# m4drat/wtf

Measured on AMD Instinct MI355X. Metric: execs/sec + emulated instr/s per node (tlv_server, HEVD) at 1/2/4/8 GPUs, higher is better.
Workload: dtype u64

## Files before the change

include/wtfgpu.h:

```cpp
#ifndef WTFGPU_H
#define WTFGPU_H

#include <stdint.h>
#include <stddef.h>

#ifdef __cplusplus
extern "C" {
#endif

#define WTFGPU_ABI_VERSION 4
#define WTFGPU_PAGE_SIZE 4096u

#define WTFGPU_OK 0
#define WTFGPU_ERR_INVALID (-1)
#define WTFGPU_ERR_NODEV (-2)
#define WTFGPU_ERR_OOM (-3)
#define WTFGPU_ERR_HIP (-4)
#define WTFGPU_ERR_STATE (-5)
#define WTFGPU_ERR_TRANSLATE (-6)

enum wtfgpu_status {
  WTFGPU_RUNNING = 0,
  WTFGPU_EXIT_BREAKPOINT = 1,
  WTFGPU_EXIT_TIMEOUT = 2,
// ... 57 lines not shown
  uint64_t zmmh[16][4];
  uint64_t zmm_hi[16][8];
  uint64_t k[8];
} wtfgpu_regs_t;

typedef struct wtfgpu_exit {
  uint32_t status;
  uint32_t vector;
  uint32_t error;
  uint32_t opcode;
  uint64_t addr;
  uint64_t rip;
  uint64_t icount;
} wtfgpu_exit_t;

typedef struct wtfgpu_run_stats {
  uint64_t kernel_launches;
  uint64_t group_steps;
  uint64_t lane_retired;
  double kernel_ms;
} wtfgpu_run_stats_t;

typedef struct wtfgpu_ctx wtfgpu_ctx;

int wtfgpu_abi_version(void);
int wtfgpu_device_count(void);
int wtfgpu_create(int device, wtfgpu_ctx **out);
int wtfgpu_destroy(wtfgpu_ctx *ctx);
void *wtfgpu_stream(wtfgpu_ctx *ctx);
int wtfgpu_select_queue(wtfgpu_ctx *ctx, uint32_t queue);
// ... 68 lines not shown
                      const wtfgpu_regs_t *in);
int wtfgpu_read_gprs(wtfgpu_ctx *ctx, uint32_t first, uint32_t count, uint64_t *out18);
int wtfgpu_write_gprs(wtfgpu_ctx *ctx, uint32_t first, uint32_t count, const uint64_t *in18);

int wtfgpu_read_exits(wtfgpu_ctx *ctx, uint32_t first, uint32_t count, wtfgpu_exit_t *out);
int wtfgpu_resume(wtfgpu_ctx *ctx, const uint32_t *lanes, uint32_t n, const uint8_t *skip_bp);
int wtfgpu_stop(wtfgpu_ctx *ctx, const uint32_t *lanes, uint32_t n, uint32_t status);

int wtfgpu_run(wtfgpu_ctx *ctx, uint32_t first, uint32_t count, uint64_t max_steps,
               wtfgpu_run_stats_t *stats);
int wtfgpu_run_async(wtfgpu_ctx *ctx, uint32_t first, uint32_t count, uint64_t max_steps);
int wtfgpu_run_wait(wtfgpu_ctx *ctx, wtfgpu_run_stats_t *stats);

int wtfgpu_prefetch_results(wtfgpu_ctx *ctx, uint32_t first, uint32_t count, wtfgpu_exit_t *exits,
                            uint64_t *bytes, uint32_t *dirty, uint64_t *stop_args);
int wtfgpu_prefetch_coverage(wtfgpu_ctx *ctx, uint32_t first, uint32_t count, uint64_t *hdr);
int wtfgpu_prefetched_coverage(wtfgpu_ctx *ctx, uint32_t *out_lanes, uint64_t *out_rips, uint64_t n);
int wtfgpu_clear_coverage_lanes(wtfgpu_ctx *ctx, const uint32_t *lanes, uint32_t n);

int wtfgpu_lane_translate(wtfgpu_ctx *ctx, uint32_t lane, uint64_t gva, uint64_t *gpa);
int wtfgpu_lane_read_phys(wtfgpu_ctx *ctx, uint32_t lane, uint64_t gpa, void *buf, uint64_t len);
int wtfgpu_lane_write_phys(wtfgpu_ctx *ctx, uint32_t lane, uint64_t gpa, const void *buf,
                           uint64_t len);
int wtfgpu_lane_read_virt(wtfgpu_ctx *ctx, uint32_t lane, uint64_t gva, void *buf, uint64_t len);
int wtfgpu_lane_write_virt(wtfgpu_ctx *ctx, uint32_t lane, uint64_t gva, const void *buf,
                           uint64_t len);

typedef struct wtfgpu_write {
  uint32_t lane;
  uint32_t len;
  uint64_t gva;
// ... 56 lines not shown
```

wtf_amd/abi.py:

```python
from __future__ import annotations

import ctypes as C
import os

HERE = os.path.dirname(os.path.abspath(__file__))
LIB_PATH = os.environ.get("WTFGPU_LIB") or os.path.join(HERE, "csrc", "libwtfgpu.so")
HOST_LIB_PATH = os.path.join(HERE, "host", "libwtf_host.so")

RUNNING, EXIT_BREAKPOINT, EXIT_TIMEOUT, EXIT_INT3, EXIT_HLT, EXIT_FAULT, EXIT_UNIMPLEMENTED, \
    EXIT_CR3, EXIT_OVERLAY_FULL, EXIT_STOPPED, EXIT_IDLE, EXIT_STOP_OK, EXIT_FEED_FAULT, EXIT_STOP_ARGS = range(14)
STATUS_NAMES = ["running", "breakpoint", "timeout", "int3", "hlt", "fault", "unimplemented",
                "cr3", "overlay_full", "stopped", "idle", "stop_ok", "feed_fault"]


class Seg(C.Structure):
    _fields_ = [("base", C.c_uint64), ("limit", C.c_uint32), ("selector", C.c_uint16),
                ("attr", C.c_uint16), ("present", C.c_uint8), ("pad", C.c_uint8 * 7)]


class Regs(C.Structure):
    _fields_ = [
        ("gpr", C.c_uint64 * 16), ("rip", C.c_uint64), ("rflags", C.c_uint64),
        ("cr0", C.c_uint64), ("cr2", C.c_uint64), ("cr3", C.c_uint64), ("cr4", C.c_uint64),
        ("cr8", C.c_uint64), ("efer", C.c_uint64), ("xcr0", C.c_uint64),
# ... 5 lines not shown
        ("idtr_limit", C.c_uint32), ("mxcsr", C.c_uint32), ("mxcsr_mask", C.c_uint32),
        ("fpcw", C.c_uint16), ("fpsw", C.c_uint16), ("fptw", C.c_uint16), ("fpop", C.c_uint16),
        ("pad0", C.c_uint32), ("fpst", C.c_uint64 * 8), ("xmm", (C.c_uint64 * 2) * 16),
        ("ymmh", (C.c_uint64 * 2) * 16), ("fpse", C.c_uint16 * 8),
        ("zmmh", (C.c_uint64 * 4) * 16), ("zmm_hi", (C.c_uint64 * 8) * 16), ("k", C.c_uint64 * 8),
    ]


class Exit(C.Structure):
    _fields_ = [("status", C.c_uint32), ("vector", C.c_uint32), ("error", C.c_uint32),
                ("opcode", C.c_uint32), ("addr", C.c_uint64), ("rip", C.c_uint64),
                ("icount", C.c_uint64)]

    def tuple(self):
        return (self.status, self.vector, self.error, self.addr, self.rip, self.icount)


class RunStats(C.Structure):
    _fields_ = [("kernel_launches", C.c_uint64), ("group_steps", C.c_uint64),
                ("lane_retired", C.c_uint64), ("kernel_ms", C.c_double)]


class BpAction(C.Structure):
    _fields_ = [("gva", C.c_uint64), ("kind", C.c_uint32), ("pad", C.c_uint32),
                ("value", C.c_uint64), ("gprs", C.c_uint64 * 17)]


BPACT_HOST, BPACT_RETURN, BPACT_SET_GPRS, BPACT_FEED = 0, 1, 2, 3
ATTRIB_ALL = 1

# ... 57 lines not shown
        "wtfgpu_apply_phys_writes": ([P, C.POINTER(Write), U32, C.c_char_p, U64, C.POINTER(I32)], C.c_int),
        "wtfgpu_restore_lanes": ([P, C.POINTER(U32), U32], C.c_int),
        "wtfgpu_set_initial_state": ([P, C.POINTER(Regs)], C.c_int),
        "wtfgpu_set_limit": ([P, U64], C.c_int),
        "wtfgpu_set_regroup": ([P, U64], C.c_int),
        "wtfgpu_set_edges": ([P, C.c_int], C.c_int),
        "wtfgpu_set_trace": ([P, U32], C.c_int),
        "wtfgpu_read_trace": ([P, U32, C.POINTER(U64), U64, C.POINTER(U64)], C.c_int),
        "wtfgpu_read_stop_args": ([P, C.POINTER(U32), U32, C.POINTER(U64)], C.c_int),
        "wtfgpu_select_queue": ([P, U32], C.c_int),
        "wtfgpu_lane_seeds": ([P, C.POINTER(U32), U32, C.POINTER(U64), C.c_int], C.c_int),
        "wtfgpu_run_async": ([P, U32, U32, U64], C.c_int),
        "wtfgpu_run_wait": ([P, C.POINTER(RunStats)], C.c_int),
        "wtfgpu_prefetch_results": ([P, U32, U32, C.POINTER(Exit), C.POINTER(U64), C.POINTER(U32), C.POINTER(U64)],
                                    C.c_int),
        "wtfgpu_prefetch_coverage": ([P, U32, U32, C.POINTER(U64)], C.c_int),
        "wtfgpu_prefetched_coverage": ([P, C.POINTER(U32), C.POINTER(U64), U64], C.c_int),
        "wtfgpu_clear_coverage_lanes": ([P, C.POINTER(U32), U32], C.c_int),
        "wtfgpu_set_breakpoints": ([P, C.POINTER(U64), U32], C.c_int),
        "wtfgpu_set_breakpoint_actions": ([P, C.POINTER(BpAction), U32], C.c_int),
        "wtfgpu_set_feed": ([P, U32, U32, C.POINTER(U64), C.c_char_p, C.c_char_p, U64], C.c_int),
        "wtfgpu_set_code_pages": ([P, C.POINTER(U64), U32], C.c_int),
        "wtfgpu_restore": ([P, U32, U32], C.c_int),
        "wtfgpu_read_regs": ([P, U32, U32, C.POINTER(Regs)], C.c_int),
        "wtfgpu_write_regs": ([P, U32, U32, C.POINTER(Regs)], C.c_int),
        "wtfgpu_read_gprs": ([P, U32, U32, C.POINTER(U64)], C.c_int),
        "wtfgpu_write_gprs": ([P, U32, U32, C.POINTER(U64)], C.c_int),
        "wtfgpu_read_exits": ([P, U32, U32, C.POINTER(Exit)], C.c_int),
        "wtfgpu_resume": ([P, C.POINTER(U32), U32, C.POINTER(C.c_uint8)], C.c_int),
        "wtfgpu_inject_fault": ([P, C.POINTER(U32), U32, U32, U32, C.POINTER(U64), C.POINTER(C.c_int32)], C.c_int),
# ... 37 lines not shown
```

wtf_amd/csrc/engine.hip:

```cpp
#include <hip/hip_runtime.h>
#include <hipcub/device/device_radix_sort.hpp>
#include <hipcub/device/device_scan.hpp>

#include <algorithm>
#include <cstddef>
#include <cstdio>
#include <cstdlib>
#include <cstring>
#include <new>
#include <vector>

#include "engine_run.h"
#include "engine_kernels.h"
#include "engine_ptmark.h"

using namespace wtfgpu_dev;

#define HIPCHK(x)                                                                        \
  do {                                                                                   \
    hipError_t e_ = (x);                                                                 \
    if (e_ != hipSuccess) {                                                              \
      fprintf(stderr, "wtfgpu: %s failed: %s (%s:%d)\n", #x, hipGetErrorString(e_), __FILE__, \
              __LINE__);                                                                 \
      return WTFGPU_ERR_HIP;                                                             \
// ... 9 lines not shown
  u64 stage_bytes = 0;
  u64 *d_stat = nullptr;
  hipEvent_t ev0 = nullptr, ev1 = nullptr;
  u32 *d_rkeys = nullptr, *d_rkeys2 = nullptr, *d_rlanes = nullptr;
  void *d_rtemp = nullptr;
  size_t rtemp_bytes = 0;
  u32 async_launches = 0;
  u8 rg_used = 2;
  u8 *h_ring = nullptr;
  u64 ring_cap = 0, ring_off = 0;
  wtfgpu_exit_t *d_exq = nullptr;
  u64 exq_cap = 0;
  u8 *d_pcov = nullptr;
  hipEvent_t ev_pre = nullptr;
  bool pre_valid = false;
};

struct wtfgpu_ctx {
  int device = 0;
  Dev P{};
  u8 *d_pool = nullptr;
  u32 *d_pfnmap = nullptr;
  u32 *d_ptbits = nullptr;
  u64 npool = 0;
  u64 *d_gpr = nullptr, *d_rip = nullptr, *d_rflags = nullptr, *d_fsb = nullptr, *d_gsb = nullptr,
      *d_icount = nullptr, *d_nbytes = nullptr;
  u32 *d_status = nullptr, *d_lflags = nullptr, *d_ovcount = nullptr, *d_ovgpfn = nullptr;
  ExitInfo *d_exinfo = nullptr;
  LaneSys *d_sys = nullptr;
  u32 *d_guc = nullptr;
// ... 77 lines not shown
int ensure_scratch(wtfgpu_ctx *c, u64 bytes) {
  QueueRes &q = *c->q;
  if (q.scratch_bytes >= bytes) return WTFGPU_OK;
  const u64 want = std::max<u64>(std::max<u64>(bytes, 2 * q.scratch_bytes), 1ull << 20);
  if (q.d_scratch) HIPCHK(hipFreeAsync(q.d_scratch, q.stream));
  q.d_scratch = nullptr;
  q.scratch_bytes = 0;
  if (hipMallocAsync((void **)&q.d_scratch, want, q.stream) != hipSuccess) return WTFGPU_ERR_OOM;
  q.scratch_bytes = want;
  return WTFGPU_OK;
}

u8 *ring_put(wtfgpu_ctx *c, const void *src, u64 bytes) {
  QueueRes &q = *c->q;
  const u64 need = (bytes + 255) & ~255ull;
  if (q.ring_off + need > q.ring_cap) {
    if (hipStreamSynchronize(q.stream) != hipSuccess) return nullptr;
    q.ring_off = 0;
    if (need > q.ring_cap) {
      if (q.h_ring) (void)hipHostFree(q.h_ring);
      q.h_ring = nullptr;
      q.ring_cap = 0;
      const u64 want = std::max<u64>(need * 2, 4ull << 20);
      if (hipHostMalloc((void **)&q.h_ring, want, hipHostMallocDefault) != hipSuccess) return nullptr;
      q.ring_cap = want;
    }
  }
  u8 *p = q.h_ring + q.ring_off;
  if (src && bytes) memcpy(p, src, bytes);
  q.ring_off += need;
  return p;
}
void ring_reset(wtfgpu_ctx *c) { c->q->ring_off = 0; }

int queue_create(QueueRes &q, u32 index) {
  q.index = index;
  HIPCHK(hipStreamCreateWithFlags(&q.stream, hipStreamNonBlocking));
  HIPCHK(hipEventCreate(&q.ev0));
  HIPCHK(hipEventCreate(&q.ev1));
  HIPCHK(hipEventCreateWithFlags(&q.ev_pre, hipEventDisableTiming));
  if (dalloc(&q.d_stat, STAT_N)) return WTFGPU_ERR_OOM;
  return WTFGPU_OK;
}
void regroup_free(QueueRes &q) {
  dfree(q.d_rkeys);
  dfree(q.d_rkeys2);
  dfree(q.d_rlanes);
  dfree(q.d_rtemp);
  q.rtemp_bytes = 0;
}
void queue_destroy(QueueRes &q) {
  if (q.stream) (void)hipStreamSynchronize(q.stream);
  regroup_free(q);
  dfree(q.d_stat);
  dfree(q.d_scratch);
  dfree(q.d_exq);
  dfree(q.d_pcov);
  if (q.h_stage) (void)hipHostFree(q.h_stage);
  q.h_stage = nullptr;
  if (q.h_ring) (void)hipHostFree(q.h_ring);
  q.h_ring = nullptr;
  if (q.ev_pre) (void)hipEventDestroy(q.ev_pre);
  if (q.ev0) (void)hipEventDestroy(q.ev0);
  if (q.ev1) (void)hipEventDestroy(q.ev1);
  if (q.stream) (void)hipStreamDestroy(q.stream);
  q = QueueRes{};
}

u64 hmix(u64 x) {
  x ^= x >> 33;
  x *= 0xff51afd7ed558ccdull;
  x ^= x >> 33;
  x *= 0xc4ceb9fe1a85ec53ull;
  x ^= x >> 33;
  return x;
}

// ... 1057 lines not shown
  if (!lanes_ok(c, first, count) || (first % c->P.lpw) || max_steps == 0 || max_steps > (1ull << 32))
    return WTFGPU_ERR_INVALID;
  if (!c->P.pool) return WTFGPU_ERR_STATE;
  if (c->q->async_launches) return WTFGPU_ERR_STATE;
  HIPCHK(hipSetDevice(c->device));
  const u64 regroup = regroup_now(c, count);
  const u64 chunk = regroup ? regroup : max_steps;
  if (regroup)
    if (int rc = regroup_buffers(c)) return rc;
  const Dev Q = run_params(c, regroup != 0);
  HIPCHK(hipEventRecord(c->q->ev_pre, c->q->stream));
  c->q->pre_valid = true;
  u64 done = 0;
  u32 k = 0;
  if (int rc = queue_launches(c, Q, first, count, chunk, max_steps, ~0ull, regroup != 0, done, k)) return rc;
  c->q->async_launches = k;
  return WTFGPU_OK;
}

int wtfgpu_run_wait(wtfgpu_ctx *c, wtfgpu_run_stats_t *stats) {
  if (!c) return WTFGPU_ERR_INVALID;
  wtfgpu_run_stats_t st{};
  if (c->q->async_launches) {
    HIPCHK(hipSetDevice(c->device));
    u64 running = 0;
    if (int rc = collect_stats(c, c->q->async_launches, st, running)) return rc;
    ring_reset(c);
    c->q->async_launches = 0;
    regroup_observe(c, st.group_steps, st.lane_retired);
  }
  if (stats) *stats = st;
  return WTFGPU_OK;
}

int wtfgpu_prefetch_results(wtfgpu_ctx *c, uint32_t first, uint32_t count, wtfgpu_exit_t *exits, uint64_t *bytes,
                            uint32_t *dirty, uint64_t *stop_args) {
  if (!lanes_ok(c, first, count) || !exits) return WTFGPU_ERR_INVALID;
  if (count == 0) return WTFGPU_OK;
  HIPCHK(hipSetDevice(c->device));
  if (c->q->exq_cap < count) {
    if (c->q->d_exq) HIPCHK(hipFreeAsync(c->q->d_exq, c->q->stream));
    c->q->d_exq = nullptr;
    c->q->exq_cap = 0;
    if (hipMallocAsync((void **)&c->q->d_exq, (u64)count * sizeof(wtfgpu_exit_t), c->q->stream) != hipSuccess)
      return WTFGPU_ERR_OOM;
    c->q->exq_cap = count;
  }
  k_pack_exits<<<(count + 255) / 256, 256, 0, c->q->stream>>>(c->P, first, count, c->q->d_exq);
  HIPCHK(hipGetLastError());
  HIPCHK(hipMemcpyAsync(exits, c->q->d_exq, (u64)count * sizeof(wtfgpu_exit_t), hipMemcpyDeviceToHost, c->q->stream));
  if (bytes) HIPCHK(hipMemcpyAsync(bytes, c->d_nbytes + first, (u64)count * 8, hipMemcpyDeviceToHost, c->q->stream));
  if (dirty) HIPCHK(hipMemcpyAsync(dirty, c->d_ovcount + first, (u64)count * 4, hipMemcpyDeviceToHost, c->q->stream));
  if (stop_args && c->d_stopargs)
    HIPCHK(hipMemcpyAsync(stop_args, c->d_stopargs + (u64)first * 6, (u64)count * 48, hipMemcpyDeviceToHost,
                          c->q->stream));
  return WTFGPU_OK;
}

constexpr u64 kPcovCap = 1ull << 22;
constexpr u64 kPcovLanes = 256, kPcovRips = kPcovLanes + kPcovCap * 4;

int wtfgpu_prefetch_coverage(wtfgpu_ctx *c, uint32_t first, uint32_t count, uint64_t *hdr) {
  if (!lanes_ok(c, first, count) || !hdr) return WTFGPU_ERR_INVALID;
  if (!c->d_covrip || count == 0) {
    hdr[0] = hdr[1] = 0;
    return WTFGPU_ERR_STATE;
  }
  HIPCHK(hipSetDevice(c->device));
  if (!c->q->d_pcov && hipMallocAsync((void **)&c->q->d_pcov, kPcovRips + kPcovCap * 8, c->q->stream) != hipSuccess) {
    c->q->d_pcov = nullptr;
    return WTFGPU_ERR_OOM;
  }
  HIPCHK(hipMemsetAsync(c->q->d_pcov, 0, 16, c->q->stream));
  k_cov_collect_stopped<<<(count + 3) / 4, 256, 0, c->q->stream>>>(
      c->P, first, count, (u32 *)(c->q->d_pcov + kPcovLanes), (u64 *)(c->q->d_pcov + kPcovRips), kPcovCap,
      (unsigned long long *)c->q->d_pcov, (u32 *)(c->q->d_pcov + 8));
  HIPCHK(hipGetLastError());
  HIPCHK(hipMemcpyAsync(hdr, c->q->d_pcov, 16, hipMemcpyDeviceToHost, c->q->stream));
  return WTFGPU_OK;
}

int wtfgpu_prefetched_coverage(wtfgpu_ctx *c, uint32_t *out_lanes, uint64_t *out_rips, uint64_t n) {
  if (!c || (n && (!out_lanes || !out_rips)) || n > kPcovCap || (n && !c->q->d_pcov)) return WTFGPU_ERR_INVALID;
  if (n == 0) return WTFGPU_OK;
  HIPCHK(hipSetDevice(c->device));
  HIPCHK(hipMemcpyAsync(out_lanes, c->q->d_pcov + kPcovLanes, n * 4, hipMemcpyDeviceToHost, c->q->stream));
  HIPCHK(hipMemcpyAsync(out_rips, c->q->d_pcov + kPcovRips, n * 8, hipMemcpyDeviceToHost, c->q->stream));
  HIPCHK(hipStreamSynchronize(c->q->stream));
  return WTFGPU_OK;
}

int wtfgpu_clear_coverage_lanes(wtfgpu_ctx *c, const uint32_t *lanes, uint32_t n) {
  if (!c || (n && !lanes)) return WTFGPU_ERR_INVALID;
// ... 646 lines not shown
```

wtf_amd/csrc/engine_device.h:

```cpp
#pragma once
#ifndef WTFGPU_HOST_SIM
#include <hip/hip_runtime.h>
#else
#include "../../tests/native/host_sim_shim.h"
#endif
#include <stdint.h>
#include "../../include/wtfgpu.h"

namespace wtfgpu_dev {

typedef uint64_t u64;
typedef uint32_t u32;
typedef uint16_t u16;
typedef uint8_t u8;
typedef int64_t i64;
typedef int32_t i32;

constexpr u64 F_CF = 0x1, F_PF = 0x4, F_AF = 0x10, F_ZF = 0x40, F_SF = 0x80, F_TF = 0x100,
              F_IF = 0x200, F_DF = 0x400, F_OF = 0x800;
constexpr u64 F_STATUS = F_CF | F_PF | F_AF | F_ZF | F_SF | F_OF;
constexpr u64 EMPTY_KEY = ~0ull;

constexpr u64 T_W = 1, T_U = 2, T_NX = 4, T_PRIV = 8, T_PT = 16;
constexpr int TLB_N = 4;
// ... 2 lines not shown
  u64 cr0, cr3, cr4, efer;
  u64 star, lstar, sfmask, kgs;
  u64 idtr, tss, cr2;
  u64 deliv_icount;
  u32 idtr_limit, pad;
  u32 cpl;
  u16 cs, ss;
};

struct LaneTlb {
  u64 tv[TLB_N], td[TLB_N];
  u64 cvpn, cptr, bloom;
  u32 tnext, pad;
};

struct ExitInfo {
  u32 vector, error, opcode, cpl;
  u64 addr;
};

struct Dev {
  const u8 *pool;
  const u32 *pfn_map;
  u64 pfn_map_len;
  u64 npool;
  const u32 *ptbits;
  u32 nlanes;
  u32 K;
  u32 lpw;
  u64 *gpr;
  u64 *rip, *rflags, *fs_base, *gs_base, *icount, *nbytes;
  u32 *status, *lflags;
  ExitInfo *exinfo;
  LaneSys *sys;
// ... 85 lines not shown
```

wtf_amd/host/gpu_backend.cc:

```cpp
#include "gpu_backend.h"
#include "module_instances.h"

#include <algorithm>
#include <chrono>
#include <cstdio>
#include <cstring>

#include "host_pool.h"

#include "blake3_lite.h"

namespace wtfgpu_host {

thread_local uint32_t GpuBackend_t::cur_ = 0;
thread_local uint64_t GpuBackend_t::servicing_bp_ = ~0ull;
thread_local uint64_t GpuBackend_t::servicing_sp_ = ~0ull;
thread_local bool GpuBackend_t::scouting_ = false;

namespace {
constexpr uint64_t kFeedRegion = 16384;
using Clock = std::chrono::steady_clock;
double ms_since(Clock::time_point t0) {
  return std::chrono::duration<double, std::milli>(Clock::now() - t0).count();
}
// ... 15 lines not shown
    case Registers_t::R12: return WTFGPU_R12;
    case Registers_t::R13: return WTFGPU_R13;
    case Registers_t::R14: return WTFGPU_R14;
    case Registers_t::R15: return WTFGPU_R15;
    case Registers_t::Rip: return 16;
    case Registers_t::Rflags: return 17;
    default: return -1;
  }
}

}

GpuBackend_t::GpuBackend_t() = default;
GpuBackend_t::~GpuBackend_t() {
  for (Part &P : parts_)
    for (void *p : {(void *)P.pin, (void *)P.ex, (void *)P.nb, (void *)P.dc, (void *)P.sargs, (void *)P.cov_hdr})
      if (p) wtfgpu_host_free(ctx_, p);
  if (wpin_) wtfgpu_host_free(ctx_, wpin_);
  if (ctx_) wtfgpu_destroy(ctx_);
}

bool GpuBackend_t::LoadDump(const std::string &dump_path) { return dump_.Parse(dump_path); }

bool GpuBackend_t::Initialize(const Options_t &Opts, const CpuState_t &CpuState) {
  if (dump_.PageCount() == 0 && !Opts.DumpPath.empty() && !LoadDump(Opts.DumpPath.string())) {
    printf("Failed to parse the dump %s\n", Opts.DumpPath.string().c_str());
    return false;
  }
  if (wtfgpu_create(Opts.GpuDevice, &ctx_) != WTFGPU_OK) {
    printf("wtfgpu_create(%d) failed\n", Opts.GpuDevice);
    return false;
// ... 1357 lines not shown

uint32_t GpuBackend_t::FreeLanes() const {
  if (busy_.empty()) return parts_n() > 1 ? nlanes_ / 2 : nlanes_;
  const Part &P = parts_[next_part_];
  if (P.launched) return P.hi - P.lo;
  return (uint32_t)P.free.size();
}

uint32_t GpuBackend_t::parts_n() const {
  if (!parts_.empty()) return (uint32_t)parts_.size();
  const char *e = getenv("WTFGPU_STREAM_PARTS");
  const uint32_t want = e ? (uint32_t)atoi(e) : 2;
  return (want >= 2 && nlanes_ >= 256 && nlanes_ % 128 == 0) ? 2 : 1;
}

bool GpuBackend_t::StreamStep(const Target_t &Target, const std::vector<StreamTestcase_t> &In, uint64_t Slice,
                              std::vector<StreamResult_t> &Out, ModuleSlots *Slots, size_t *Taken) {
  const auto t0 = Clock::now();
  if (Taken) *Taken = 0;
  if (busy_.empty()) {
    busy_.assign(nlanes_, 0);
    tag_.assign(nlanes_, 0);
    tc_bytes_.assign(nlanes_, 0);
    lres_.assign(nlanes_, LaneResult{});
    plain_.assign(nlanes_, 0);
    const uint32_t n = parts_n();
    done_.assign((nlanes_ + n - 1) / n + 1, 0);
    parts_.assign(n, Part{});
    for (uint32_t p = 0; p < n; p++) {
      Part &Q = parts_[p];
      Q.lo = (uint32_t)((uint64_t)nlanes_ * p / n);
      Q.hi = (uint32_t)((uint64_t)nlanes_ * (p + 1) / n);
      Q.free.resize(Q.hi - Q.lo);
      for (uint32_t l = Q.lo; l < Q.hi; l++) Q.free[l - Q.lo] = l;
    }
    std::vector<uint32_t> all(nlanes_);
    for (uint32_t l = 0; l < nlanes_; l++) all[l] = l;
    if (wtfgpu_stop(ctx_, all.data(), nlanes_, WTFGPU_EXIT_IDLE)) return false;
  }
  const bool pipelined = parts_.size() > 1;
  const uint32_t pi = next_part_;
  next_part_ = (next_part_ + 1) % (uint32_t)parts_.size();
  Part &P = parts_[pi];
  if (pipelined && wtfgpu_select_queue(ctx_, pi)) return false;
  if (pipelined && P.launched && !harvest_part(P, Target, Out, Slots)) return false;
  const auto ti = Clock::now();
  stats_.harvest_ms += std::chrono::duration<double, std::milli>(ti - t0).count();
  std::vector<uint32_t> &fresh = fresh_;
  {
    const size_t take = std::min(In.size(), P.free.size());
    fresh.assign(P.free.begin(), P.free.begin() + (std::ptrdiff_t)take);
    P.free.erase(P.free.begin(), P.free.begin() + (std::ptrdiff_t)take);
  }
  if (Taken) *Taken = fresh.size();
  stats_.fresh_ms += ms_since(ti);
  if (!fresh.empty()) {
    if (wtfgpu_restore_lanes(ctx_, fresh.data(), (uint32_t)fresh.size())) return false;
    stats_.restore_dev_ms += ms_since(ti);
    const size_t n = fresh.size();
// ... 8 lines not shown
    }
    HostPool::Get().For(chunks, 1, [&](size_t c) {
      RefillChunk &C = rchunks_[c];
      C.call.clear();
      C.pre.clear();
      C.bytes = 0;
      const size_t hi = std::min(n, (c + 1) * kChunk);
      for (size_t i = c * kChunk; i < hi; i++) {
        const uint32_t l = fresh[i];
        if (touched_[l]) reset_view(l);
        PrepFeed f{};
        busy_[l] = 1;
        tag_[l] = In[i].tag;
        tc_bytes_[l] = In[i].size;
        const StreamTestcase_t &T = In[i];
        bool prepared = true;
        switch (T.prep) {
          case PreparedInsert_t::Call: prepared = false; break;
          case PreparedInsert_t::Failed:
            view(l).result = Crash_t("insert-testcase-failed");
            C.pre.push_back(l);
            break;
          case PreparedInsert_t::Nothing: break;
          case PreparedInsert_t::Feed:
            if (!feed_action_ || T.prep_size > kFeedRegion)
              prepared = false;
            else
              f = PrepFeed{T.prep_data, (uint32_t)T.prep_size, 1, 0};
            break;
          case PreparedInsert_t::Insert:
            if (!insert_action_ || T.size + 4 > kFeedRegion)
              prepared = false;
            else
              f = PrepFeed{T.data, (uint32_t)T.size, 1, 1};
            break;
        }
        pf_[l] = f;
        flen_[i] = f.has ? f.len + (f.ins ? 4 : 0) : 0;
        fhas_[i] = f.has;
        C.bytes += flen_[i];
        if (!prepared) {
          C.call.push_back((uint32_t)i);
          continue;
        }
        if (Slots) Slots->ResetLane(l);
      }
    }, n >= 512);
    recycle_arenas();
    const auto tm = Clock::now();
    stats_.restore_ms += std::chrono::duration<double, std::milli>(tm - ti).count();
// ... 24 lines not shown
      for (size_t k = 0; k < call_.size(); k++) {
        const uint32_t i = call_[k], l = call[k];
        if (!touched_[l]) continue;
        const LaneView &v = views_[l];
        flen_[i] = (uint32_t)v.feed.size();
        fhas_[i] = v.has_feed;
        rchunks_[i / kChunk].bytes += flen_[i];
        if (v.result.has_value()) pre_call.push_back(l);
      }
      if (!pre_call.empty()) {
        tmp_lanes_.resize(pre_.size() + pre_call.size());
        std::merge(pre_.begin(), pre_.end(), pre_call.begin(), pre_call.end(), tmp_lanes_.begin());
        pre_.swap(tmp_lanes_);
      }
    }
    if (feeds) {
      const auto tf = Clock::now();
      uint64_t total = 0;
      for (size_t c = 0; c < chunks; c++) {
        const uint64_t b = rchunks_[c].bytes;
        rchunks_[c].bytes = total;
        total += b;
      }
      foff_[n] = total;
      if (total > P.pin_cap) {
        if (P.pin) wtfgpu_host_free(ctx_, P.pin);
        P.pin = nullptr;
        P.pin_cap = std::max<uint64_t>(total * 2, 1 << 20);
        void *p = nullptr;
        if (wtfgpu_host_alloc(ctx_, P.pin_cap, &p)) return false;
        P.pin = (uint8_t *)p;
      }
      HostPool::Get().For(chunks, 1, [&](size_t c) {
        uint64_t at = rchunks_[c].bytes;
        const size_t hi = std::min(n, (c + 1) * kChunk);
        for (size_t i = c * kChunk; i < hi; i++) {
          foff_[i] = at;
          if (!flen_[i]) continue;
          const uint32_t l = fresh[i];
          const PrepFeed &f = pf_[l];
          uint8_t *o = P.pin + at;
          if (f.has) {
            if (f.ins) {
              memcpy(o, &f.len, 4);
              o += 4;
            }
            if (f.len) memcpy(o, f.p, f.len);
          } else {
            memcpy(o, views_[l].feed.data(), flen_[i]);
          }
          at += flen_[i];
        }
      }, n >= 512);
      if (wtfgpu_set_feed_lanes(ctx_, fresh.data(), (uint32_t)n, foff_.data(), fhas_.data(), P.pin, total))
        return false;
      stats_.up_feed_ms += ms_since(tf);
    }
    if (!pre_.empty() && wtfgpu_stop(ctx_, pre_.data(), (uint32_t)pre_.size(), WTFGPU_EXIT_STOPPED) != WTFGPU_OK)
      return false;
    stats_.upload_ms += ms_since(tu);
    stats_.testcases += fresh.size();
  }
  stats_.insert_ms += ms_since(ti);
  const auto to = Clock::now();
  if (P.occ.empty()) {
    P.occ.swap(fresh);
  } else if (!fresh.empty()) {
    tmp_lanes_.resize(P.occ.size() + fresh.size());
    std::merge(P.occ.begin(), P.occ.end(), fresh.begin(), fresh.end(), tmp_lanes_.begin());
// ... 18 lines not shown
    if (p) return true;
    void *q = nullptr;
    if (wtfgpu_host_alloc(ctx_, bytes, &q)) return false;
    p = (std::remove_reference_t<decltype(p)>)q;
    return true;
  };
  if (P.ex_cap < count) {
    if (P.ex) wtfgpu_host_free(ctx_, P.ex);
    P.ex = nullptr;
    P.ex_cap = 0;
    if (!grow(P.ex, (uint64_t)count * sizeof(wtfgpu_exit_t))) return false;
    P.ex_cap = count;
  }
  const bool args = !args_results_.empty();
  if (!grow(P.nb, (uint64_t)count * 8) || !grow(P.dc, (uint64_t)count * 4) || !grow(P.cov_hdr, 16) ||
      (args && !grow(P.sargs, (uint64_t)count * 48)))
    return false;
  if (wtfgpu_prefetch_results(ctx_, P.lo, count, P.ex, P.nb, P.dc, args ? P.sargs : nullptr) != WTFGPU_OK)
    return false;
  P.pf_cov = !full_coverage_ && !device_attrib_ && wtfgpu_prefetch_coverage(ctx_, P.lo, count, P.cov_hdr) == WTFGPU_OK;
  return true;
}

bool GpuBackend_t::harvest_part(Part &P, const Target_t &Target, std::vector<StreamResult_t> &Out,
                                ModuleSlots *Slots) {
  const auto tw = Clock::now();
  wtfgpu_run_stats_t rs{};
  if (wtfgpu_run_wait(ctx_, &rs)) return false;
  const auto te = Clock::now();
  stats_.run_ms += std::chrono::duration<double, std::milli>(te - tw).count();
  account_run(rs);
  P.launched = false;
  const uint32_t first = P.lo, count = P.hi - P.lo;
// ... 25 lines not shown
  const wtfgpu_exit_t *ex = P.ex;
  const size_t n = P.occ.size();
  constexpr size_t kChunk = 2048;
  const size_t chunks = (n + kChunk - 1) / kChunk;
  if (hchunks_.size() < chunks) hchunks_.resize(chunks);
  const bool fill = !want_gprs_;
  HostPool::Get().For(chunks, 1, [&](size_t c) {
    HarvestChunk &C = hchunks_[c];
    C.fin.clear();
    C.used.clear();
    C.run.clear();
    C.hits.clear();
    C.named.clear();
    uint64_t bytes = 0;
    const size_t hi = std::min(n, (c + 1) * kChunk);
    for (size_t i = c * kChunk; i < hi; i++) {
      const uint32_t l = P.occ[i];
      const wtfgpu_exit_t &e = ex[l - first];
      LaneView &v = views_[l];
      const auto mark = [&]() -> LaneView & {
        touched_[l] = 1;
        return v;
      };
      bool plain = false, direct = false;
      const auto ends = [&](TestcaseResult_t &&R) {
        if (fill && !touched_[l]) {
          lres_[l].result = std::move(R);
          direct = true;
        } else {
          mark().result = std::move(R);
// ... 95 lines not shown
  P.occ.swap(run_);
  if (finished.empty()) return true;
  if (!fill && !fill_lanes(finished, first, ex, lres_)) return false;
  const auto tc = Clock::now();
  if (pf) {
    stats_.alg_bytes += b_exec;
  } else {
    uint32_t lo = finished.front() & ~63u, hi = finished.back() + 1;
    std::vector<uint64_t> nb(hi - lo);
    std::vector<uint32_t> dc(hi - lo);
    if (wtfgpu_read_bytes(ctx_, lo, hi - lo, nb.data()) == WTFGPU_OK &&
        wtfgpu_read_dirty_counts(ctx_, lo, hi - lo, dc.data()) == WTFGPU_OK)
      for (uint32_t l : finished) stats_.alg_bytes += nb[l - lo] + 2ull * 4096 * dc[l - lo] + tc_bytes_[l];
  }
  stats_.bytes_ms += ms_since(tc);
  collect_coverage(finished, lres_, pf && P.pf_cov ? P.cov_hdr : nullptr);
  {
    uint32_t last = ~0u;
    size_t added = 0;
    for (const std::pair<uint32_t, uint64_t> &E : cov_sorted_) {
      const uint32_t l = E.first;
      if (l == last) continue;
      last = l;
      if (!plain_[l] || lres_[l].new_coverage.empty()) continue;
      plain_[l] = 0;
      fill_lane(l, ex[l - first], lres_[l]);
      P.res_used.push_back(l);
      added++;
    }
    if (added) std::inplace_merge(P.res_used.begin(), P.res_used.end() - (std::ptrdiff_t)added, P.res_used.end());
// ... 146 lines not shown
```

wtf_amd/host/gpu_backend.h:

```cpp
#pragma once
#include "unimpl_hist.h"
#include <atomic>
#include <memory>
#include <mutex>
#include <shared_mutex>
#include <string>
#include <unordered_map>
#include <vector>

#include "../../include/wtfgpu.h"
#include "kdmp.h"
#include "module_slots.h"
#include "runner.h"
#include "wtf_api.h"

namespace wtfgpu_host {

struct BatchStats {
  uint64_t rounds = 0, breakpoint_hits = 0, kernel_launches = 0, retired = 0, group_steps = 0;
  uint64_t page_fetches = 0, prefetched_pages = 0, batches = 0, testcases = 0, staged_pages = 0, stack_windows = 0;
  uint64_t prepared = 0;
  double kernel_ms = 0, service_ms = 0, total_ms = 0;
  double bulk_ms = 0, prefetch_ms = 0, handler_ms = 0, fetch_ms = 0, flush_ms = 0;
  double insert_ms = 0, coverage_ms = 0, target_restore_ms = 0;
// ... 180 lines not shown
  std::vector<uint64_t> cov_rips_;
  std::vector<uint8_t> cov_want_;
  std::vector<std::pair<uint32_t, uint64_t>> cov_sorted_;
  bool cov_ovf_warned_ = false;
  bool want_gprs_ = true;
  uint64_t last_icount_ = 0;
  LaneResult last_run_;
  bool last_error_ = false;
  struct Part {
    uint32_t lo = 0, hi = 0;
    bool launched = false;
    std::vector<uint32_t> occ, free;
    std::vector<uint32_t> res_used;
    wtfgpu_exit_t *ex = nullptr;
    uint64_t ex_cap = 0;
    uint8_t *pin = nullptr;
    uint64_t pin_cap = 0;
    bool pf = false, pf_cov = false;
    uint64_t *nb = nullptr, *sargs = nullptr, *cov_hdr = nullptr;
    uint32_t *dc = nullptr;
  };
  bool prefetch_part(Part &P);
  std::vector<Part> parts_;
  uint8_t *wpin_ = nullptr;
  uint64_t wpin_cap_ = 0;
  uint32_t next_part_ = 0;
  uint32_t parts_n() const;
  bool harvest_part(Part &P, const Target_t &Target, std::vector<StreamResult_t> &Out, ModuleSlots *Slots);
  void finish_coverage(uint32_t n, std::vector<LaneResult> *out, std::vector<uint32_t> *timedout);
  bool set_code_pages();

  wtfgpu_ctx *ctx_ = nullptr;
  KernelDump dump_;
  CpuState_t initial_{};
  wtfgpu_regs_t initial_regs_{};
  uint32_t nlanes_ = 0, overlay_pages_ = 0;
  uint32_t dirty_cap_ = 0;
  uint64_t limit_ = 0;
  mutable std::vector<LaneView> views_;
  mutable std::vector<uint8_t> touched_;
  struct PrepFeed {
    const uint8_t *p = nullptr;
    uint32_t len = 0;
    uint8_t has = 0, ins = 0;
  };
  std::vector<PrepFeed> pf_;
  static thread_local uint32_t cur_;
  std::unordered_map<uint64_t, BreakpointHandler_t> breakpoints_;
  std::vector<wtfgpu_bp_action_t> bp_actions_;
  uint32_t trace_cap_ = 0;
  uint64_t tenet_cap_ = 0;
  std::unordered_map<uint64_t, BreakpointAction_t::ArgsResult_t> args_results_;
  bool feed_action_ = false;
  bool insert_action_ = false;
  int upload_feed(uint32_t n);
  std::unordered_set<uint64_t> aggregate_;
  std::unordered_set<uint64_t> code_vpns_;
  std::vector<uint64_t> extra_new_;
  void commit_fresh(const std::vector<uint64_t> &fresh);
  std::unordered_set<Gva_t> last_new_coverage_;
  mutable BatchStats stats_;
// ... 38 lines not shown
```

Before: 15.51 million.

## Overlap host feed packing and result readback with in-flight GPU partitions

Run stats are copied into pinned host memory at launch, and run_wait now waits on a results event instead of synchronizing the whole stream. Exit results are prefetched as structure-of-arrays copies and assembled on the host per chunk. Coverage gets its own event wait. Testcase feeds are prepacked into a double-buffered pinned buffer before harvesting the previous partition, so host packing overlaps GPU work. This adds event bookkeeping and a ring_late fallback sync, and carries ordering risk if the feed buffer is reused while a copy is still in flight.

```diff
diff --git a/include/wtfgpu.h b/include/wtfgpu.h
--- a/include/wtfgpu.h
+++ b/include/wtfgpu.h
@@ -95,6 +95,14 @@
   uint64_t icount;
 } wtfgpu_exit_t;
 
+typedef struct wtfgpu_exinfo {
+  uint32_t vector;
+  uint32_t error;
+  uint32_t opcode;
+  uint32_t cpl;
+  uint64_t addr;
+} wtfgpu_exinfo_t;
+
 typedef struct wtfgpu_run_stats {
   uint64_t kernel_launches;
   uint64_t group_steps;
@@ -193,7 +201,14 @@
 
 int wtfgpu_prefetch_results(wtfgpu_ctx *ctx, uint32_t first, uint32_t count, wtfgpu_exit_t *exits,
                             uint64_t *bytes, uint32_t *dirty, uint64_t *stop_args);
+int wtfgpu_prefetch_results_soa(wtfgpu_ctx *ctx, uint32_t first, uint32_t count, uint32_t *status, uint64_t *rip,
+                                uint64_t *icount, wtfgpu_exinfo_t *exinfo, uint64_t *bytes, uint32_t *dirty,
+                                uint64_t *stop_args);
+int wtfgpu_assemble_exits(const uint32_t *status, const uint64_t *rip, const uint64_t *icount,
+                          const wtfgpu_exinfo_t *exinfo, const uint32_t *lanes, uint32_t first, uint32_t n,
+                          wtfgpu_exit_t *out);
 int wtfgpu_prefetch_coverage(wtfgpu_ctx *ctx, uint32_t first, uint32_t count, uint64_t *hdr);
+int wtfgpu_prefetch_coverage_wait(wtfgpu_ctx *ctx);
 int wtfgpu_prefetched_coverage(wtfgpu_ctx *ctx, uint32_t *out_lanes, uint64_t *out_rips, uint64_t n);
 int wtfgpu_clear_coverage_lanes(wtfgpu_ctx *ctx, const uint32_t *lanes, uint32_t n);
 
diff --git a/wtf_amd/abi.py b/wtf_amd/abi.py
--- a/wtf_amd/abi.py
+++ b/wtf_amd/abi.py
@@ -43,6 +43,11 @@
 
     def tuple(self):
         return (self.status, self.vector, self.error, self.addr, self.rip, self.icount)
+
+
+class ExInfo(C.Structure):
+    _fields_ = [("vector", C.c_uint32), ("error", C.c_uint32), ("opcode", C.c_uint32), ("cpl", C.c_uint32),
+                ("addr", C.c_uint64)]
 
 
 class RunStats(C.Structure):
@@ -130,6 +135,11 @@
         "wtfgpu_run_wait": ([P, C.POINTER(RunStats)], C.c_int),
         "wtfgpu_prefetch_results": ([P, U32, U32, C.POINTER(Exit), C.POINTER(U64), C.POINTER(U32), C.POINTER(U64)],
                                     C.c_int),
+        "wtfgpu_prefetch_results_soa": ([P, U32, U32, C.POINTER(U32), C.POINTER(U64), C.POINTER(U64),
+                                         C.POINTER(ExInfo), C.POINTER(U64), C.POINTER(U32), C.POINTER(U64)], C.c_int),
+        "wtfgpu_assemble_exits": ([C.POINTER(U32), C.POINTER(U64), C.POINTER(U64), C.POINTER(ExInfo),
+                                   C.POINTER(U32), U32, U32, C.POINTER(Exit)], C.c_int),
+        "wtfgpu_prefetch_coverage_wait": ([P], C.c_int),
         "wtfgpu_prefetch_coverage": ([P, U32, U32, C.POINTER(U64)], C.c_int),
         "wtfgpu_prefetched_coverage": ([P, C.POINTER(U32), C.POINTER(U64), U64], C.c_int),
         "wtfgpu_clear_coverage_lanes": ([P, C.POINTER(U32), U32], C.c_int),
diff --git a/wtf_amd/csrc/engine.hip b/wtf_amd/csrc/engine.hip
--- a/wtf_amd/csrc/engine.hip
+++ b/wtf_amd/csrc/engine.hip
@@ -47,6 +47,10 @@
   u8 *d_pcov = nullptr;
   hipEvent_t ev_pre = nullptr;
   bool pre_valid = false;
+  hipEvent_t ev_res = nullptr, ev_cov = nullptr;
+  bool res_pending = false, cov_pending = false;
+  bool ring_late = false;
+  u64 *h_stat = nullptr;
 };
 
 struct wtfgpu_ctx {
@@ -154,9 +158,11 @@
 u8 *ring_put(wtfgpu_ctx *c, const void *src, u64 bytes) {
   QueueRes &q = *c->q;
   const u64 need = (bytes + 255) & ~255ull;
+  if (q.async_launches) q.ring_late = true;
   if (q.ring_off + need > q.ring_cap) {
     if (hipStreamSynchronize(q.stream) != hipSuccess) return nullptr;
     q.ring_off = 0;
+    q.ring_late = false;
     if (need > q.ring_cap) {
       if (q.h_ring) (void)hipHostFree(q.h_ring);
       q.h_ring = nullptr;
@@ -179,7 +185,10 @@
   HIPCHK(hipEventCreate(&q.ev0));
   HIPCHK(hipEventCreate(&q.ev1));
   HIPCHK(hipEventCreateWithFlags(&q.ev_pre, hipEventDisableTiming));
+  HIPCHK(hipEventCreateWithFlags(&q.ev_res, hipEventDisableTiming));
+  HIPCHK(hipEventCreateWithFlags(&q.ev_cov, hipEventDisableTiming));
   if (dalloc(&q.d_stat, STAT_N)) return WTFGPU_ERR_OOM;
+  HIPCHK(hipHostMalloc((void **)&q.h_stat, STAT_N * 8, hipHostMallocDefault));
   return WTFGPU_OK;
 }
 void regroup_free(QueueRes &q) {
@@ -200,7 +209,11 @@
   q.h_stage = nullptr;
   if (q.h_ring) (void)hipHostFree(q.h_ring);
   q.h_ring = nullptr;
+  if (q.h_stat) (void)hipHostFree(q.h_stat);
+  q.h_stat = nullptr;
   if (q.ev_pre) (void)hipEventDestroy(q.ev_pre);
+  if (q.ev_res) (void)hipEventDestroy(q.ev_res);
+  if (q.ev_cov) (void)hipEventDestroy(q.ev_cov);
   if (q.ev0) (void)hipEventDestroy(q.ev0);
   if (q.ev1) (void)hipEventDestroy(q.ev1);
   if (q.stream) (void)hipStreamDestroy(q.stream);
@@ -1288,19 +1301,33 @@
   u64 done = 0;
   u32 k = 0;
   if (int rc = queue_launches(c, Q, first, count, chunk, max_steps, ~0ull, regroup != 0, done, k)) return rc;
+  HIPCHK(hipMemcpyAsync(c->q->h_stat, c->q->d_stat, STAT_N * 8, hipMemcpyDeviceToHost, c->q->stream));
   c->q->async_launches = k;
+  c->q->res_pending = false;
   return WTFGPU_OK;
 }
 
 int wtfgpu_run_wait(wtfgpu_ctx *c, wtfgpu_run_stats_t *stats) {
   if (!c) return WTFGPU_ERR_INVALID;
   wtfgpu_run_stats_t st{};
-  if (c->q->async_launches) {
+  QueueRes &q = *c->q;
+  if (q.async_launches) {
     HIPCHK(hipSetDevice(c->device));
-    u64 running = 0;
-    if (int rc = collect_stats(c, c->q->async_launches, st, running)) return rc;
+    if (q.res_pending) HIPCHK(hipEventSynchronize(q.ev_res));
+    else HIPCHK(hipStreamSynchronize(q.stream));
+    q.res_pending = false;
+    float ms = 0;
+    HIPCHK(hipEventElapsedTime(&ms, q.ev0, q.ev1));
+    const u64 *s = q.h_stat;
+    st.kernel_launches = q.async_launches;
+    st.group_steps = s[0];
+    st.lane_retired = s[1];
+    st.kernel_ms = ms;
+    print_stamps(s);
+    if (q.ring_late) HIPCHK(hipStreamSynchronize(q.stream));
+    q.ring_late = false;
     ring_reset(c);
-    c->q->async_launches = 0;
+    q.async_launches = 0;
     regroup_observe(c, st.group_steps, st.lane_retired);
   }
   if (stats) *stats = st;
@@ -1328,6 +1355,56 @@
   if (stop_args && c->d_stopargs)
     HIPCHK(hipMemcpyAsync(stop_args, c->d_stopargs + (u64)first * 6, (u64)count * 48, hipMemcpyDeviceToHost,
                           c->q->stream));
+  HIPCHK(hipEventRecord(c->q->ev_res, c->q->stream));
+  c->q->res_pending = c->q->async_launches != 0;
+  return WTFGPU_OK;
+}
+
+int wtfgpu_prefetch_results_soa(wtfgpu_ctx *c, uint32_t first, uint32_t count, uint32_t *status, uint64_t *rip,
+                                uint64_t *icount, wtfgpu_exinfo_t *exinfo, uint64_t *bytes, uint32_t *dirty,
+                                uint64_t *stop_args) {
+  if (!lanes_ok(c, first, count) || !status || !rip || !icount || !exinfo) return WTFGPU_ERR_INVALID;
+  if (count == 0) return WTFGPU_OK;
+  HIPCHK(hipSetDevice(c->device));
+  hipStream_t s = c->q->stream;
+  HIPCHK(hipMemcpyAsync(status, c->d_status + first, (u64)count * 4, hipMemcpyDeviceToHost, s));
+  HIPCHK(hipMemcpyAsync(rip, c->d_rip + first, (u64)count * 8, hipMemcpyDeviceToHost, s));
+  HIPCHK(hipMemcpyAsync(icount, c->d_icount + first, (u64)count * 8, hipMemcpyDeviceToHost, s));
+  HIPCHK(hipMemcpyAsync(exinfo, c->d_exinfo + first, (u64)count * sizeof(ExitInfo), hipMemcpyDeviceToHost, s));
+  if (bytes) HIPCHK(hipMemcpyAsync(bytes, c->d_nbytes + first, (u64)count * 8, hipMemcpyDeviceToHost, s));
+  if (dirty) HIPCHK(hipMemcpyAsync(dirty, c->d_ovcount + first, (u64)count * 4, hipMemcpyDeviceToHost, s));
+  if (stop_args && c->d_stopargs)
+    HIPCHK(hipMemcpyAsync(stop_args, c->d_stopargs + (u64)first * 6, (u64)count * 48, hipMemcpyDeviceToHost, s));
+  HIPCHK(hipEventRecord(c->q->ev_res, s));
+  c->q->res_pending = c->q->async_launches != 0;
+  return WTFGPU_OK;
+}
+
+int wtfgpu_assemble_exits(const uint32_t *status, const uint64_t *rip, const uint64_t *icount,
+                          const wtfgpu_exinfo_t *exinfo, const uint32_t *lanes, uint32_t first, uint32_t n,
+                          wtfgpu_exit_t *out) {
+  if (!status || !rip || !icount || !exinfo || (n && !out)) return WTFGPU_ERR_INVALID;
+  for (uint32_t i = 0; i < n; i++) {
+    const uint32_t lane = lanes ? lanes[i] : first + i;
+    if (lane < first) return WTFGPU_ERR_INVALID;
+    const uint32_t k = lane - first;
+    wtfgpu_exit_t e;
+    e.status = status[k];
+    e.vector = e.error = e.opcode = 0;
+    e.addr = 0;
+    if (e.status == WTFGPU_EXIT_FAULT) {
+      const wtfgpu_exinfo_t &x = exinfo[k];
+      e.vector = x.vector;
+      e.error = x.error;
+      e.addr = x.addr;
+      e.opcode = x.cpl;
+    } else if (e.status == WTFGPU_EXIT_UNIMPLEMENTED) {
+      e.opcode = exinfo[k].opcode;
+    }
+    e.rip = rip[k];
+    e.icount = icount[k];
+    out[k] = e;
+  }
   return WTFGPU_OK;
 }
 
@@ -1351,6 +1428,17 @@
       (unsigned long long *)c->q->d_pcov, (u32 *)(c->q->d_pcov + 8));
   HIPCHK(hipGetLastError());
   HIPCHK(hipMemcpyAsync(hdr, c->q->d_pcov, 16, hipMemcpyDeviceToHost, c->q->stream));
+  HIPCHK(hipEventRecord(c->q->ev_cov, c->q->stream));
+  c->q->cov_pending = true;
+  return WTFGPU_OK;
+}
+
+int wtfgpu_prefetch_coverage_wait(wtfgpu_ctx *c) {
+  if (!c) return WTFGPU_ERR_INVALID;
+  if (!c->q->cov_pending) return WTFGPU_OK;
+  HIPCHK(hipSetDevice(c->device));
+  HIPCHK(hipEventSynchronize(c->q->ev_cov));
+  c->q->cov_pending = false;
   return WTFGPU_OK;
 }
 
diff --git a/wtf_amd/csrc/engine_device.h b/wtf_amd/csrc/engine_device.h
--- a/wtf_amd/csrc/engine_device.h
+++ b/wtf_amd/csrc/engine_device.h
@@ -40,10 +40,8 @@
   u32 tnext, pad;
 };
 
-struct ExitInfo {
-  u32 vector, error, opcode, cpl;
-  u64 addr;
-};
+typedef wtfgpu_exinfo_t ExitInfo;
+static_assert(sizeof(ExitInfo) == 24, "wtfgpu_exinfo_t: 4 x u32 + u64");
 
 struct Dev {
   const u8 *pool;
diff --git a/wtf_amd/host/gpu_backend.cc b/wtf_amd/host/gpu_backend.cc
--- a/wtf_amd/host/gpu_backend.cc
+++ b/wtf_amd/host/gpu_backend.cc
@@ -53,7 +53,8 @@
 GpuBackend_t::GpuBackend_t() = default;
 GpuBackend_t::~GpuBackend_t() {
   for (Part &P : parts_)
-    for (void *p : {(void *)P.pin, (void *)P.ex, (void *)P.nb, (void *)P.dc, (void *)P.sargs, (void *)P.cov_hdr})
+    for (void *p : {(void *)P.pin[0], (void *)P.pin[1], (void *)P.ex, (void *)P.nb, (void *)P.dc, (void *)P.sargs, (void *)P.cov_hdr,
+                    (void *)P.xst, (void *)P.xrip, (void *)P.xic, (void *)P.xinfo})
       if (p) wtfgpu_host_free(ctx_, p);
   if (wpin_) wtfgpu_host_free(ctx_, wpin_);
   if (ctx_) wtfgpu_destroy(ctx_);
@@ -1441,6 +1442,91 @@
   return (want >= 2 && nlanes_ >= 256 && nlanes_ % 128 == 0) ? 2 : 1;
 }
 
+bool GpuBackend_t::prepared_feed(const StreamTestcase_t &T, PrepFeed &f) const {
+  switch (T.prep) {
+    case PreparedInsert_t::Call: return false;
+    case PreparedInsert_t::Failed:
+    case PreparedInsert_t::Nothing: return true;
+    case PreparedInsert_t::Feed:
+      if (!feed_action_ || T.prep_size > kFeedRegion) return false;
+      f = PrepFeed{T.prep_data, (uint32_t)T.prep_size, 1, 0};
+      return true;
+    case PreparedInsert_t::Insert:
+      if (!insert_action_ || T.size + 4 > kFeedRegion) return false;
+      f = PrepFeed{T.data, (uint32_t)T.size, 1, 1};
+      return true;
+  }
+  return false;
+}
+
+uint8_t *GpuBackend_t::feed_buffer(Part &P, uint64_t bytes) {
+  P.pin_k ^= 1;
+  const uint32_t k = P.pin_k;
+  if (bytes > P.pin_cap[k] || !P.pin[k]) {
+    if (P.pin[k]) wtfgpu_host_free(ctx_, P.pin[k]);
+    P.pin[k] = nullptr;
+    P.pin_cap[k] = std::max<uint64_t>(bytes * 2, 1 << 20);
+    void *p = nullptr;
+    if (wtfgpu_host_alloc(ctx_, P.pin_cap[k], &p)) {
+      P.pin_cap[k] = 0;
+      return nullptr;
+    }
+    P.pin[k] = (uint8_t *)p;
+  }
+  return P.pin[k];
+}
+
+bool GpuBackend_t::prepack_feeds(Part &P, const std::vector<StreamTestcase_t> &In) {
+  const size_t n = In.size();
+  if (!n) return false;
+  constexpr size_t kChunk = 1024;
+  const size_t chunks = (n + kChunk - 1) / kChunk;
+  if (poff_.size() < n + 1) poff_.resize(n + 1);
+  pchunk_.assign(chunks, 0);
+  std::atomic<bool> all{true};
+  HostPool::Get().For(chunks, 1, [&](size_t c) {
+    uint64_t bytes = 0;
+    const size_t hi = std::min(n, (c + 1) * kChunk);
+    for (size_t i = c * kChunk; i < hi; i++) {
+      PrepFeed f{};
+      if (!prepared_feed(In[i], f)) {
+        all = false;
+        return;
+      }
+      bytes += f.has ? f.len + (f.ins ? 4 : 0) : 0;
+    }
+    pchunk_[c] = bytes;
+  }, n >= 512);
+  if (!all) return false;
+  uint64_t total = 0;
+  for (size_t c = 0; c < chunks; c++) {
+    const uint64_t b = pchunk_[c];
+    pchunk_[c] = total;
+    total += b;
+  }
+  uint8_t *const pin = feed_buffer(P, total);
+  if (!pin) return false;
+  poff_[n] = total;
+  HostPool::Get().For(chunks, 1, [&](size_t c) {
+    uint64_t at = pchunk_[c];
+    const size_t hi = std::min(n, (c + 1) * kChunk);
+    for (size_t i = c * kChunk; i < hi; i++) {
+      poff_[i] = at;
+      PrepFeed f{};
+      prepared_feed(In[i], f);
+      if (!f.has) continue;
+      uint8_t *o = pin + at;
+      if (f.ins) {
+        memcpy(o, &f.len, 4);
+        o += 4;
+      }
+      if (f.len) memcpy(o, f.p, f.len);
+      at += f.len + (f.ins ? 4 : 0);
+    }
+  }, n >= 512);
+  return true;
+}
+
 bool GpuBackend_t::StreamStep(const Target_t &Target, const std::vector<StreamTestcase_t> &In, uint64_t Slice,
                               std::vector<StreamResult_t> &Out, ModuleSlots *Slots, size_t *Taken) {
   const auto t0 = Clock::now();
@@ -1470,6 +1556,7 @@
   next_part_ = (next_part_ + 1) % (uint32_t)parts_.size();
   Part &P = parts_[pi];
   if (pipelined && wtfgpu_select_queue(ctx_, pi)) return false;
+  const bool packed = pipelined && P.launched && (feed_action_ || insert_action_) && prepack_feeds(P, In);
   if (pipelined && P.launched && !harvest_part(P, Target, Out, Slots)) return false;
   const auto ti = Clock::now();
   stats_.harvest_ms += std::chrono::duration<double, std::milli>(ti - t0).count();
@@ -1508,26 +1595,10 @@
         tag_[l] = In[i].tag;
         tc_bytes_[l] = In[i].size;
         const StreamTestcase_t &T = In[i];
-        bool prepared = true;
-        switch (T.prep) {
-          case PreparedInsert_t::Call: prepared = false; break;
-          case PreparedInsert_t::Failed:
-            view(l).result = Crash_t("insert-testcase-failed");
-            C.pre.push_back(l);
-            break;
-          case PreparedInsert_t::Nothing: break;
-          case PreparedInsert_t::Feed:
-            if (!feed_action_ || T.prep_size > kFeedRegion)
-              prepared = false;
-            else
-              f = PrepFeed{T.prep_data, (uint32_t)T.prep_size, 1, 0};
-            break;
-          case PreparedInsert_t::Insert:
-            if (!insert_action_ || T.size + 4 > kFeedRegion)
-              prepared = false;
-            else
-              f = PrepFeed{T.data, (uint32_t)T.size, 1, 1};
-            break;
+        const bool prepared = prepared_feed(T, f);
+        if (T.prep == PreparedInsert_t::Failed) {
+          view(l).result = Crash_t("insert-testcase-failed");
+          C.pre.push_back(l);
         }
         pf_[l] = f;
         flen_[i] = f.has ? f.len + (f.ins ? 4 : 0) : 0;
@@ -1582,7 +1653,12 @@
         pre_.swap(tmp_lanes_);
       }
     }
-    if (feeds) {
+    if (feeds && packed) {
+      const auto tf = Clock::now();
+      if (wtfgpu_set_feed_lanes(ctx_, fresh.data(), (uint32_t)n, poff_.data(), fhas_.data(), P.pin[P.pin_k], poff_[n]))
+        return false;
+      stats_.up_feed_ms += ms_since(tf);
+    } else if (feeds) {
       const auto tf = Clock::now();
       uint64_t total = 0;
       for (size_t c = 0; c < chunks; c++) {
@@ -1591,14 +1667,8 @@
         total += b;
       }
       foff_[n] = total;
-      if (total > P.pin_cap) {
-        if (P.pin) wtfgpu_host_free(ctx_, P.pin);
-        P.pin = nullptr;
-        P.pin_cap = std::max<uint64_t>(total * 2, 1 << 20);
-        void *p = nullptr;
-        if (wtfgpu_host_alloc(ctx_, P.pin_cap, &p)) return false;
-        P.pin = (uint8_t *)p;
-      }
+      uint8_t *const pin = feed_buffer(P, total);
+      if (!pin) return false;
       HostPool::Get().For(chunks, 1, [&](size_t c) {
         uint64_t at = rchunks_[c].bytes;
         const size_t hi = std::min(n, (c + 1) * kChunk);
@@ -1607,7 +1677,7 @@
           if (!flen_[i]) continue;
           const uint32_t l = fresh[i];
           const PrepFeed &f = pf_[l];
-          uint8_t *o = P.pin + at;
+          uint8_t *o = pin + at;
           if (f.has) {
             if (f.ins) {
               memcpy(o, &f.len, 4);
@@ -1620,7 +1690,7 @@
           at += flen_[i];
         }
       }, n >= 512);
-      if (wtfgpu_set_feed_lanes(ctx_, fresh.data(), (uint32_t)n, foff_.data(), fhas_.data(), P.pin, total))
+      if (wtfgpu_set_feed_lanes(ctx_, fresh.data(), (uint32_t)n, foff_.data(), fhas_.data(), pin, total))
         return false;
       stats_.up_feed_ms += ms_since(tf);
     }
@@ -1669,9 +1739,11 @@
   }
   const bool args = !args_results_.empty();
   if (!grow(P.nb, (uint64_t)count * 8) || !grow(P.dc, (uint64_t)count * 4) || !grow(P.cov_hdr, 16) ||
-      (args && !grow(P.sargs, (uint64_t)count * 48)))
+      !grow(P.xst, (uint64_t)count * 4) || !grow(P.xrip, (uint64_t)count * 8) || !grow(P.xic, (uint64_t)count * 8) ||
+      !grow(P.xinfo, (uint64_t)count * sizeof(wtfgpu_exinfo_t)) || (args && !grow(P.sargs, (uint64_t)count * 48)))
     return false;
-  if (wtfgpu_prefetch_results(ctx_, P.lo, count, P.ex, P.nb, P.dc, args ? P.sargs : nullptr) != WTFGPU_OK)
+  if (wtfgpu_prefetch_results_soa(ctx_, P.lo, count, P.xst, P.xrip, P.xic, P.xinfo, P.nb, P.dc,
+                                  args ? P.sargs : nullptr) != WTFGPU_OK)
     return false;
   P.pf_cov = !full_coverage_ && !device_attrib_ && wtfgpu_prefetch_coverage(ctx_, P.lo, count, P.cov_hdr) == WTFGPU_OK;
   return true;
@@ -1727,6 +1799,9 @@
     C.named.clear();
     uint64_t bytes = 0;
     const size_t hi = std::min(n, (c + 1) * kChunk);
+    if (pf)
+      wtfgpu_assemble_exits(P.xst, P.xrip, P.xic, P.xinfo, &P.occ[c * kChunk], first, (uint32_t)(hi - c * kChunk),
+                            P.ex);
     for (size_t i = c * kChunk; i < hi; i++) {
       const uint32_t l = P.occ[i];
       const wtfgpu_exit_t &e = ex[l - first];
@@ -1852,6 +1927,7 @@
       for (uint32_t l : finished) stats_.alg_bytes += nb[l - lo] + 2ull * 4096 * dc[l - lo] + tc_bytes_[l];
   }
   stats_.bytes_ms += ms_since(tc);
+  if (pf && P.pf_cov && wtfgpu_prefetch_coverage_wait(ctx_)) return false;
   collect_coverage(finished, lres_, pf && P.pf_cov ? P.cov_hdr : nullptr);
   {
     uint32_t last = ~0u;
diff --git a/wtf_amd/host/gpu_backend.h b/wtf_amd/host/gpu_backend.h
--- a/wtf_amd/host/gpu_backend.h
+++ b/wtf_amd/host/gpu_backend.h
@@ -218,13 +218,20 @@
     std::vector<uint32_t> res_used;
     wtfgpu_exit_t *ex = nullptr;
     uint64_t ex_cap = 0;
-    uint8_t *pin = nullptr;
-    uint64_t pin_cap = 0;
+    uint32_t *xst = nullptr;
+    uint64_t *xrip = nullptr, *xic = nullptr;
+    wtfgpu_exinfo_t *xinfo = nullptr;
+    uint8_t *pin[2] = {nullptr, nullptr};
+    uint64_t pin_cap[2] = {0, 0};
+    uint32_t pin_k = 0;
     bool pf = false, pf_cov = false;
     uint64_t *nb = nullptr, *sargs = nullptr, *cov_hdr = nullptr;
     uint32_t *dc = nullptr;
   };
   bool prefetch_part(Part &P);
+  uint8_t *feed_buffer(Part &P, uint64_t bytes);
+  bool prepack_feeds(Part &P, const std::vector<StreamTestcase_t> &In);
+  std::vector<uint64_t> poff_, pchunk_;
   std::vector<Part> parts_;
   uint8_t *wpin_ = nullptr;
   uint64_t wpin_cap_ = 0;
@@ -249,6 +256,7 @@
     uint8_t has = 0, ins = 0;
   };
   std::vector<PrepFeed> pf_;
+  bool prepared_feed(const StreamTestcase_t &T, PrepFeed &f) const;
   static thread_local uint32_t cur_;
   std::unordered_map<uint64_t, BreakpointHandler_t> breakpoints_;
   std::vector<wtfgpu_bp_action_t> bp_actions_;
```

After: 15.86 million, median of 4. 1.02x the previous value.
